# gear-genomics/tracy

Hardware: AMD Instinct MI355X
Metric: GCUPS (tracy align: Gotoh affine-gap DP cells per second, whole job) (higher is better)
Workload: dtype int16 (score sweeps) / int32 (tracebacks)

## Files before the change

### tracy_amd/csrc/pipe_kernels.h

```cpp
#ifndef TRACY_AMD_PIPE_KERNELS_H
#define TRACY_AMD_PIPE_KERNELS_H

#include <hip/hip_runtime.h>

#include "capi_internal.h"
#include "stream_plan.h"

namespace {
using namespace tracyhip;

__global__ __launch_bounds__(64) void trim_kernel(const uint8_t* __restrict__ ops, const uint64_t* __restrict__ ops_off,
                                                  const uint32_t* __restrict__ ops_len, const uint32_t* __restrict__ ref_len,
                                                  const uint8_t* __restrict__ forward, const uint32_t* __restrict__ trim_left,
                                                  const uint32_t* __restrict__ trim_right, uint32_t ntraces, TrimRec* __restrict__ out) {
  const uint32_t t = blockIdx.x;
  if (t >= ntraces) return;
  const uint8_t* o = ops + ops_off[t];
  const uint32_t L = ops_len[t];
  const uint32_t lane = threadIdx.x;
  int32_t s = -1, e = -1;
  for (uint32_t base = 0; base < L; base += 64) {
    const uint32_t j = base + lane;
    const bool hit = (j < L) && (o[L - 1 - j] != 'h');
    const unsigned long long m = __ballot(hit);
// ... 136 lines not shown
      b[j] = (uint8_t)c;
      if (c >= 4u) { f |= c >= 5u ? 2 : 4; any = true; }
    }
    if (cnt == kCqBytesPerThread) __builtin_memcpy(out + i0, b, kCqBytesPerThread);
    else for (uint32_t j = 0; j < cnt; ++j) out[i0 + j] = b[j];
    if (any && special) { special[i0 >> 8] = 1; special[(i0 + cnt - 1) >> 8] = 1; }
  }
  if (f) atomicOr(flag, f);
}
__global__ void cq_rows_kernel(const uint8_t* __restrict__ in, uint64_t n, int32_t* flag) {
  const uint64_t i0 = ((uint64_t)blockIdx.x * blockDim.x + threadIdx.x) * kCqBytesPerThread;
  if (i0 >= n) return;
  const uint32_t cnt = n - i0 < kCqBytesPerThread ? (uint32_t)(n - i0) : kCqBytesPerThread;
  uint8_t b[kCqBytesPerThread];
  if (cnt == kCqBytesPerThread) __builtin_memcpy(b, in + i0, kCqBytesPerThread);
  else for (uint32_t j = 0; j < cnt; ++j) b[j] = in[i0 + j];
  bool bad = false;
#pragma unroll
  for (uint32_t j = 0; j < kCqBytesPerThread; ++j)
    if (j < cnt && !cq_row_char(b[j])) bad = true;
  if (bad) atomicOr(flag, 1);
}

__device__ __forceinline__ uint32_t encode_word(uint32_t w, uint32_t cnt, bool& any_special, bool& invalid) {
  uint32_t codes = 0;
#pragma unroll
  for (uint32_t j = 0; j < 4u; ++j) {
    const uint8_t ch = (uint8_t)(w >> (8 * j));
    const uint8_t up = ch & 0xdfu;
    const uint32_t c = up == 'A' ? 0u : up == 'C' ? 1u : up == 'G' ? 2u : up == 'T' ? 3u : up == 'N' ? 4u : 5u;
    if (j < cnt) {
      invalid |= !(ch == 'A' || ch == 'C' || ch == 'G' || ch == 'T' || ch == 'N');
      any_special |= c >= 4u;
    }
    codes |= c << (8 * j);
  }
  return codes;
}
__global__ __launch_bounds__(256) void encode_codes_kernel(const uint8_t* __restrict__ in, uint8_t* __restrict__ out, uint64_t n,
                                                           uint8_t* __restrict__ special, int32_t* __restrict__ verr) {
  const uint64_t i0 = ((uint64_t)blockIdx.x * blockDim.x + threadIdx.x) * 16u;
  if (i0 >= n) return;
  bool any_special = false, invalid = false;
  if (n - i0 >= 16u) {
    uint32_t w[4];
    __builtin_memcpy(w, in + i0, 16);
#pragma unroll
    for (int q = 0; q < 4; ++q) w[q] = encode_word(w[q], 4u, any_special, invalid);
    __builtin_memcpy(out + i0, w, 16);
  } else {
    for (uint64_t i = i0; i < n; i += 4) {
      const uint32_t cnt = (n - i < 4u) ? (uint32_t)(n - i) : 4u;
      uint32_t w = 0;
      for (uint32_t j = 0; j < cnt; ++j) w |= (uint32_t)in[i + j] << (8 * j);
      const uint32_t c = encode_word(w, cnt, any_special, invalid);
      for (uint32_t j = 0; j < cnt; ++j) out[i + j] = (uint8_t)(c >> (8 * j));
    }
  }
  if (any_special) special[i0 >> 8] = 1;
  if (verr && invalid) atomicOr(verr, 4);
}

struct VoteDesc { uint64_t a1_off, a2_off; uint32_t stride, m, n, pad; };
constexpr int kVoteK = 11;
constexpr uint32_t kVoteBits = 1u << 16;
constexpr uint32_t kVotePiece = 65, kVoteTile = 64 * kVotePiece;
__device__ inline uint32_t vote_hash(uint32_t kmer) { return (kmer * 0x9E3779B1u) >> 16; }
__global__ __launch_bounds__(64) void kmer_vote_kernel(const VoteDesc* __restrict__ desc, const float* __restrict__ prof,
                                                       const uint8_t* __restrict__ codes, uint32_t* __restrict__ votes) {
  __shared__ uint32_t bm[2][kVoteBits / 32];
  __shared__ uint8_t cons[1040];
  __shared__ __attribute__((aligned(16))) uint8_t win[kVoteTile + 16];
  const VoteDesc d = desc[blockIdx.x];
  const uint32_t lane = threadIdx.x;
  uint32_t hf = 0, hr = 0;
  const uint32_t m = d.m < 1024u ? d.m : 1024u;
  if (m >= (uint32_t)kVoteK && d.n >= (uint32_t)kVoteK) {
    for (uint32_t i = lane; i < kVoteBits / 32; i += 64) { bm[0][i] = 0; bm[1][i] = 0; }
    constexpr uint32_t kCols = 8;
    for (uint32_t j0 = 0; j0 < m; j0 += 64 * kCols) {
      float v[kCols][4];
#pragma unroll
      for (uint32_t u = 0; u < kCols; ++u) {
// ... 83 lines not shown
```

### tracy_amd/csrc/pipeline.hip

```cpp
#include <hip/hip_runtime.h>

#include <algorithm>
#include <cstdlib>
#include <cstring>
#include <numeric>
#include <string>
#include <thread>
#include <vector>

#include "../../include/tracy_hip.h"
#include "capi_internal.h"
#include "launch.h"
#include "pipe_internal.h"
#include "pipe_kernels.h"
#include "stream_fields.h"

using namespace tracyhip;

namespace {
void reset_call_stats(tracyhip_ctx* ctx, uint32_t ntraces) {
  ctx->stats = tracyhip_call_stats{};
  ctx->stats.traces = ntraces;
  for (auto* l : ctx->lanes) l->stats = tracyhip_call_stats{};
}
// ... 719 lines not shown
  std::vector<B16TableDesc> td;
  bool b16 = false;
  OrientOut oo;
  std::vector<TrimRec> h_trim;
  void *d_final_sc = nullptr, *d_ops = nullptr, *d_olen = nullptr;
  uint64_t ops_total = 0;

  AlignRun(tracyhip_ctx* c, const tracyhip_align_job* j, const tracyhip_params* q, int m, const tracyhip_align_result* o)
      : ctx(c), job(j), prm(q), mem(m), out(o), nt(j->ntraces), sp(j->profiles), sr(j->refs), st(c->stream), p(*q), trims(trims_of(j)) {
    p.hfree = 1;
    p.vfree = 0;
  }

  int setup() {
    int rc;
    const uint64_t ep = seqset_extent(sp), er = seqset_extent(sr);
    if ((rc = stage_in(ctx, ctx->dev[DB_IN1], sp.data, ep * 4, mem, &d_prof))) return rc;
    if ((rc = stage_in(ctx, ctx->dev[DB_IN2], sr.data, er, mem, &d_ref))) return rc;
    HIP_TRY(ctx->dev[DB_ERR].ensure(kErrBytes));
    HIP_TRY(hipMemsetAsync(ctx->dev[DB_ERR].p, 0, kErrBytes, st));
    d_verr = static_cast<int32_t*>(ctx->dev[DB_ERR].p) + kErrVerdictWord;
    HIP_TRY(ctx->ensure_codes(er ? er : 1, st));
    if (er) {
      hipLaunchKernelGGL(encode_codes_kernel, dim3((unsigned)((er + 4095) / 4096)), dim3(256), 0, st, static_cast<const uint8_t*>(d_ref),
                         ctx->codes(), er, ctx->special_blocks(), job->oriented ? (int32_t*)nullptr : d_verr);
      HIP_TRY(hipGetLastError());
    }
    mf.resize(nt); mt.resize(nt); tl.resize(nt); rn.resize(nt); ridx.resize(nt);
    uint64_t max_mn = 0;
    for (uint32_t t = 0; t < nt; ++t) {
      ridx[t] = job->ref_index ? job->ref_index[t] : t;
      if (ridx[t] >= sr.count) return set_error(TRACYHIP_ERR_ARG, "ref_index[%u] out of range", t);
      mf[t] = sp.length[t];
      rn[t] = sr.length[ridx[t]];
      uint32_t l = trims.left(t), r = trims.right(t);
      if ((uint64_t)l + r >= mf[t]) { l = 0; r = 0; }
      tl[t] = l;
      mt[t] = mf[t] - (l + r);
      max_mn = std::max<uint64_t>(max_mn, (uint64_t)mf[t] + rn[t]);
    }
    if ((rc = check_params(&p, max_mn))) return rc;

    return TRACYHIP_OK;
  }

  int orient() {
    int rc;
// ... 572 lines not shown
      if ((rc = stage_in(ctx, buf(), bc.signal, sext * 4, mem, &d_sig))) return rc;
      if ((rc = stage_in(ctx, buf(), bc.bcpos, bext * 4, mem, &d_pos))) return rc;
    }
    for (uint32_t t = 0; t < nt; ++t) dext = std::max<uint64_t>(dext, out->dcp_offset[t] + 2ull * dp.maxindel + 2);
    if ((rc = io(bc.primary, bext, true, &d_pri))) return rc;
    if ((rc = io(bc.secondary, bext, true, &d_sec))) return rc;
    if ((rc = io(out->bp, sizeof(BreakpointOut) * (size_t)nt, false, &d_bp))) return rc;
    if ((rc = io(out->secdecomp, bext, false, &d_sd))) return rc;
    if ((rc = io(out->fractions, sizeof(double) * 2 * (size_t)nt, false, &d_fr))) return rc;
    if ((rc = io(out->dcp_indel, dext * 4, false, &d_di))) return rc;
    if ((rc = io(out->dcp_err, dext * 4, false, &d_de))) return rc;
    if (mem == TRACYHIP_MEM_HOST) {
      HIP_TRY(hipMemsetAsync(d_di, 0, dext * 4, st));
      HIP_TRY(hipMemsetAsync(d_de, 0, dext * 4, st));
    }
    if ((rc = io(out->dstatus, sizeof(DecompOut) * (size_t)nt, false, &d_dst))) return rc;
    if ((rc = io(out->score_trim, sizeof(int32_t) * (size_t)nt, false, &d_strim))) return rc;

    HIP_TRY(ctx->dev[DB_ERR].ensure(kErrBytes));
    HIP_TRY(hipMemsetAsync(ctx->dev[DB_ERR].p, 0, kErrBytes, st));
    HIP_TRY(ctx->ensure_codes(er ? er : 1, st));
    if (er) {
      int32_t* d_verr = static_cast<int32_t*>(ctx->dev[DB_ERR].p) + kErrVerdictWord;
      hipLaunchKernelGGL(encode_codes_kernel, dim3((unsigned)((er + 4095) / 4096)), dim3(256), 0, st, static_cast<const uint8_t*>(d_ref),
                         ctx->codes(), er, ctx->special_blocks(), job->oriented ? (int32_t*)nullptr : d_verr);
      HIP_TRY(hipGetLastError());
      int32_t herr = 0;
      HIP_TRY(hipMemcpyAsync(&herr, d_verr, sizeof(int32_t), hipMemcpyDeviceToHost, st));
      HIP_TRY(ctx_sync(ctx));
      if ((herr & 4) && !wildtype) return set_error(TRACYHIP_ERR_ARG, "reference windows must be upper-case [ACGTN] (loadSingleFasta, fasta.h:54-95)");
    }

    return TRACYHIP_OK;
  }

  int orientation() {
    int rc;
    stage_clock.mark("decompose.2_orientation");
    HIP_TRY(b_sc2.ensure(sizeof(int32_t) * 2 * (size_t)nt));
    h_sc2.assign(2 * (size_t)nt, 0);
    if (!given && !shared_stages) {
      DpProblem pb;
      DpProblemLease lease(ctx, pb);
      pb.mode = MODE_PROF; pb.a1_profile = true; pb.a2_profile = true; pb.d_a1 = d_prof; pb.d_a2 = d_refprof;
      pb.desc.resize(2 * (size_t)nt); pb.k.resize(2 * (size_t)nt);
      for (uint32_t t = 0; t < nt; ++t) {
        PairDesc d = qp_desc(t, true);
// ... 868 lines not shown
```

### tracy_amd/csrc/stream.hip

```cpp
#include <hip/hip_runtime.h>

#include <algorithm>
#include <cstring>
#include <numeric>
#include <string>
#include <type_traits>
#include <vector>

#include "../../include/tracy_hip.h"
#include "capi_internal.h"
#include "decompose_launch.h"
#include "launch.h"
#include "pipe_internal.h"
#include "pipe_kernels.h"
#include "stream_fields.h"
#include "stream_plan.h"

using namespace tracyhip;

#define TRY(expr) do { const int _rc = (expr); if (_rc) return _rc; } while (0)

namespace {

struct Arena {
// ... 10 lines not shown
  void take_into(T*& p, size_t count) { p = take<T>(count); }
};

__device__ __forceinline__ void s_count(unsigned long long* lc, int which, unsigned long long v = 1ull) { atomicAdd(lc + which, v); }
template <class Body>
__device__ __forceinline__ void with_counters(unsigned long long* cnt, Body body) {
  __shared__ unsigned long long lc[SC_COUNT];
  for (uint32_t i = threadIdx.x; i < (uint32_t)SC_COUNT; i += blockDim.x) lc[i] = 0;
  __syncthreads();
  body(lc);
  __syncthreads();
  for (uint32_t i = threadIdx.x; i < (uint32_t)SC_COUNT; i += blockDim.x)
    if (lc[i]) atomicAdd(cnt + i, lc[i]);
}
__device__ __forceinline__ void s_count_front(unsigned long long* lc, const FrontDesc& f) {
  const Credit c = front_credit(f.m_rest, f.n, kFrontK1, kFrontHalfW1);
  s_count(lc, SC_FRONT_CELLS, c.cells);
  s_count(lc, SC_FRONT_BYTES, c.bytes);
}

inline int queued_prio(const tracyhip_ctx* ctx, uint32_t tier) { return ctx->queue_prio >= tier ? 1 : 0; }

__global__ void s_expand_kernel(const SGeom* __restrict__ geom, uint32_t nt, VoteDesc* __restrict__ vd, RowMaxDesc* __restrict__ rm_rest,
                                RowMaxDesc* __restrict__ rm_trim, RowMaxDesc* __restrict__ rm_full, B16TableDesc* __restrict__ td) {
  const uint32_t t = blockIdx.x * blockDim.x + threadIdx.x;
  if (t >= nt) return;
  const SGeom G = geom[t];
  const uint64_t a1 = G.prof_off + G.tl;
  vd[t] = VoteDesc{a1, G.ref_off, G.mf, G.mt, G.rn, 0u};
  rm_rest[t] = RowMaxDesc{a1, G.mf, G.mt, kFrontRows};
  rm_trim[t] = RowMaxDesc{a1, G.mf, G.mt, 0u};
  if (rm_full) rm_full[t] = RowMaxDesc{G.prof_off, G.mf, G.mf, 0u};
  td[t] = B16TableDesc{G.prof_off, G.tab_off, G.mf, G.mf, G.tab_stride, 0u};
}

__device__ __forceinline__ PairDesc s_stage1_desc(const SGeom& G, uint32_t t, uint32_t nt, uint32_t o) {
  PairDesc d{};
  d.a1_off = G.prof_off + G.tl;
  d.a1_stride = G.mf;
  d.m = G.mt;
  d.a2_off = G.ref_off;
  d.n = G.rn;
  d.a2_stride = G.rn;
  d.out = o * nt + t;
  d.flags = o ? PAIR_A2_REVCOMP : 0u;
  d.lastrow_off = G.lr_off[o];
  return d;
}

__global__ void s_orient_plan_kernel(SParams p, const SGeom* __restrict__ geom, const uint32_t* __restrict__ votes, const int32_t* __restrict__ ub,
                                     const int32_t* __restrict__ ub1, PairDesc* __restrict__ full, PairDesc* __restrict__ pre,
                                     FrontDesc* __restrict__ fd, STrace* __restrict__ tr, unsigned long long* __restrict__ cnt) {
  with_counters(cnt, [&](unsigned long long* lc) {
  const uint32_t t = blockIdx.x * blockDim.x + threadIdx.x;
  if (t >= p.nt) return;
  const SGeom G = geom[t];
  const uint32_t R = kFrontRows;
  const SOrient o = s_orient_class(votes[2 * t], votes[2 * t + 1], G.mt, (G.flags & SG_FRONT_OK) != 0u, p.exact != 0u);
  const uint32_t g = o.g, cls = o.cls;
  PairDesc fa = s_skip_pair(t), fb = s_skip_pair(t), pa = s_skip_pair(t), pb = s_skip_pair(t);
  FrontDesc f{};
  f.flags = PAIR_SKIP;
  f.out = t;
  uint64_t cells = 0, bytes = 0, pcells = 0;
  const Credit full_c = sweep_pair_credit(G.mt, G.rn, true, false), pre_c = prefix_credit(G.mt, G.rn, R);
  const uint64_t full_cells = full_c.cells, pre_cells = pre_c.cells, full_bytes = full_c.bytes;
  if (cls == 0u) {
    pa = s_stage1_desc(G, t, p.nt, g);
    pa.flags |= PAIR_KEEP_ROW;
    pcells += pre_cells;
    if (p.exact) { fa = s_stage1_desc(G, t, p.nt, 1u - g); cells += full_cells; bytes += full_bytes; }
    else { pb = s_stage1_desc(G, t, p.nt, 1u - g); pcells += pre_cells; }
    f.row_off = G.lr_off[g];
    f.a2_off = G.ref_off;
    f.tab_off = G.tab_off + G.tl + R;
    f.tab_stride = G.tab_stride;
    f.m_rest = G.mt - R;
    f.n = G.rn;
    f.flags = g ? PAIR_A2_REVCOMP : 0u;
    f.R = R;
    f.rest = ub[t];
    f.tight = (p.ge <= -2 && ub1[t] <= ub[t]) ? (uint32_t)(ub[t] - ub1[t]) + 1u : 0u;
    s_count_front(lc, f);
  } else if (cls == 1u) {
    fa = s_stage1_desc(G, t, p.nt, g);
    fb = s_stage1_desc(G, t, p.nt, 1u - g);
    cells += 2 * full_cells; bytes += 2 * full_bytes;
  } else {
    fa = s_stage1_desc(G, t, p.nt, g);
    pb = s_stage1_desc(G, t, p.nt, 1u - g);
    cells += full_cells; pcells += pre_cells; bytes += full_bytes;
  }
  if (p.split_prefix) { s_count(lc, SC_FRONT_CELLS, pcells); s_count(lc, SC_FRONT_BYTES, pcells ? pre_c.bytes : 0ull); }
  else cells += pcells;
  full[G.full_a] = fa;
  full[G.full_b] = fb;
  pre[t] = pa;
  if (!p.exact) pre[p.nt + t] = pb;
  fd[t] = f;
  STrace S{};
  S.g = (uint8_t)g;
  S.cls = (uint8_t)cls;
  tr[t] = S;
  s_count(lc, SC_SWEEP_CELLS, cells);
  s_count(lc, SC_SWEEP_BYTES, bytes);
  });
}

__device__ __forceinline__ uint32_t s_front_result(uint32_t t, const FrontOut* __restrict__ fo1, const int32_t* __restrict__ fs1, const uint32_t* __restrict__ fe1,
                                                   const FrontOut* __restrict__ fo2, const int32_t* __restrict__ fs2, const uint32_t* __restrict__ fe2, int64_t* s_g) {
  if (fo1[t].ok) { *s_g = fs1[t]; return fe1[2 * t + 1] ? fe1[2 * t + 1] + fo1[t].shift : 0u; }
  if (fo2[t].ok) { *s_g = fs2[t]; return fe2[2 * t + 1] ? fe2[2 * t + 1] + fo2[t].shift : 0u; }
  return 0u;
}

__global__ void s_orient_early_kernel(SParams p, const FrontOut* __restrict__ fo1,
                                      const int32_t* __restrict__ fs1, const uint32_t* __restrict__ fe1, const FrontOut* __restrict__ fo2,
                                      const int32_t* __restrict__ fs2, const uint32_t* __restrict__ fe2, STrace* __restrict__ tr, int prio) {
  wave_prio(prio);
  const uint32_t t = blockIdx.x * blockDim.x + threadIdx.x;
  if (t >= p.nt) return;
  STrace S = tr[t];
  if (S.cls != 0u || !p.use_votes || !p.exact) return;
  const uint32_t g = S.g;
  int64_t s_g = 0;
  const uint32_t fce = s_front_result(t, fo1, fs1, fe1, fo2, fs2, fe2, &s_g);
  if (fce == 0u) return;
  if (g == 0u) S.sc[0] = (int32_t)s_g;
  else S.sc[1] = (int32_t)s_g;
// ... 577 lines not shown
  for (int b = 0; b < 4; ++b) { ak[b].index = sc.idx + (size_t)b * n; ak[b].count = count + b; }
  if (!quads) ak[3].npairs = 0;
  TRY(timing_begin(ctx, bl.kind == 0 ? TRACYHIP_TIMER_TRACE : TRACYHIP_TIMER_ORIGIN, 0, 0));
  bool large = false;
  HIP_TRY(launch_band16_counted(bl.kind, ak[0], ak[1], ak[2], ak[3], st, (ctx->b16_fork_ok && !ctx->knobs.no_fork) ? &ctx->b16_fork : nullptr,
                                ctx->knobs.b16_multi_max, &large));
  if (large) ++sc.large_stages;
  TRY(timing_end(ctx));
  return TRACYHIP_OK;
}

uint64_t band_words_cap(uint64_t rows, uint64_t npairs, uint64_t budget_left) {
  const uint64_t worst = rows * 131 + npairs * 10240;
  return std::max<uint64_t>(std::min(worst, budget_left / 2), 1ull << 20);
}
struct OrientStage {
  const void* d_prof;
  const int16_t* d_qp;
  int32_t* d_lastrow;
  bool exact;
  PairDesc* desc_trim;
  std::function<int()> filler;
  std::function<int()> early_tail;
};
int queue_orientation(tracyhip_ctx* ctx, const tracyhip_params& p, const SParams& sp, const StreamHost& h, StreamCommon& sc, const OrientStage& os) {
  hipStream_t st = ctx->stream;
  const uint32_t nt = h.nt;
  const dim3 g256((nt + 255) / 256), b256(256);
  const float* prof = static_cast<const float*>(os.d_prof);
  hipLaunchKernelGGL(s_expand_kernel, g256, b256, 0, st, sc.geom, nt, sc.vd, sc.rm_rest, sc.rm_trim, sc.rm_full, sc.td);
  HIP_TRY(hipGetLastError());
  const bool prep_fork = ctx->b16_fork_ok && !ctx->knobs.no_fork;
  hipStream_t sp1 = st;
  if (prep_fork) {
    HIP_TRY(hipEventRecord(ctx->b16_fork.forked, st));
    HIP_TRY(hipStreamWaitEvent(ctx->b16_fork.side[1], ctx->b16_fork.forked, 0));
    sp1 = ctx->b16_fork.side[1];
    ctx->stream = sp1;
  }
  {
    int rc = timing_begin(ctx, TRACYHIP_TIMER_MISC, 0, h.tab_tot * 2);
    hipError_t e = hipSuccess;
    if (!rc) {
      e = launch_b16_tables(sc.td, nt, os.d_prof, false, p.match, p.mismatch, sub_limit(&p), kTagShift, const_cast<int16_t*>(os.d_qp),
                            static_cast<int32_t*>(ctx->dev[DB_ERR].p), sp1);
      rc = timing_end(ctx);
    }
    ctx->stream = st;
    hipLaunchKernelGGL(rowmax_rest_kernel, dim3(nt), dim3(64), 0, sp1, sc.rm_rest, prof, (float)p.match, (float)p.mismatch, sc.ub, sc.ub1);
    hipLaunchKernelGGL(rowmax_rest_kernel, dim3(nt), dim3(64), 0, sp1, sc.rm_trim, prof, (float)p.match, (float)p.mismatch, sc.top_trim, (int32_t*)nullptr);
    if (sc.rm_full) hipLaunchKernelGGL(rowmax_rest_kernel, dim3(nt), dim3(64), 0, sp1, sc.rm_full, prof, (float)p.match, (float)p.mismatch, sc.top_full, (int32_t*)nullptr);
    hipLaunchKernelGGL(kmer_vote_kernel, dim3(nt), dim3(64), 0, st, sc.vd, prof, ctx->codes(), sc.votes);
    if (prep_fork) {
      HIP_TRY(hipEventRecord(ctx->b16_fork.joined[1], sp1));
      HIP_TRY(hipStreamWaitEvent(st, ctx->b16_fork.joined[1], 0));
    }
    if (rc) return rc;
    HIP_TRY(e);
  }
  hipLaunchKernelGGL(s_orient_plan_kernel, g256, b256, 0, st, sp, sc.geom, sc.votes, sc.ub, sc.ub1, sc.full, sc.pre, sc.fd, sc.tr, sc.cnt);
  HIP_TRY(hipGetLastError());
  DpArgs a = sweep_args(ctx, p, os.d_prof, ctx->codes(), sc.sc2, os.d_lastrow);
  if (!ctx->knobs.no_compact) a.special_blocks = ctx->special_blocks();
  if (sp.use_votes) { a.votes = sc.votes; a.vote_nt = nt; }
  DpArgs ap = a;
  ap.pairs = sc.pre;
  ap.votes = nullptr;
  const uint32_t npre_all = (os.exact ? 1u : 2u) * nt;
  auto front_tiers = [&]() -> int {
    TRY(timing_begin(ctx, TRACYHIP_TIMER_FRONT, 0, 0));
    const int rc = front_tiers_run(ctx, p, sc, nt, os.d_qp, ctx->codes(), reinterpret_cast<const uint32_t*>(os.d_lastrow), h.max_rest);
    const int rc2 = timing_end(ctx);
    return rc ? rc : rc2;
  };
  if (ctx->b16_fork_ok && !ctx->knobs.no_fork) {
    const B16Fork& fk = ctx->b16_fork;
    HIP_TRY(hipEventRecord(fk.forked, st));
    HIP_TRY(hipStreamWaitEvent(fk.side[0], fk.forked, 0));
    ctx->stream = fk.side[0];
    int rc = TRACYHIP_OK;
    {
      DpArgs af = a, apl = ap;
      launch_diag_periods(ctx, &p, h.classes[0].K, 0u, npre_all, true, af, apl);
      const uint32_t tall_min = (os.exact && !ctx->knobs.no_prefix_tall_beside) ? 0u : ctx->knobs.prefix_tall_min;
      if (launch_gotoh_ckpt_front(h.classes[0].K, af, 0u, apl, npre_all, fk.side[0], tall_min) != hipSuccess) rc = set_error(TRACYHIP_ERR_HIP, "prefix launch failed");
    }
    ctx->queue_prio = ctx->knobs.chain_prio;
    if (!rc) rc = front_tiers();
    if (!rc && os.early_tail) {
      hipLaunchKernelGGL(s_orient_early_kernel, g256, b256, 0, fk.side[0], sp, sc.fo1, sc.fs1, sc.fe1, sc.fo2, sc.fs2, sc.fe2, sc.tr, queued_prio(ctx, 1));
      if (hipGetLastError() != hipSuccess) rc = set_error(TRACYHIP_ERR_HIP, "early decision launch failed");
      else rc = os.early_tail();
    }
    ctx->queue_prio = 0;
    ctx->stream = st;
    HIP_TRY(hipEventRecord(fk.joined[0], fk.side[0]));
    if (rc) {
      HIP_TRY(hipStreamWaitEvent(st, fk.joined[0], 0));
      return rc;
    }
    if (ctx->knobs.sweeps_alone) HIP_TRY(hipStreamWaitEvent(st, fk.joined[0], 0));
    auto sweeps = [&]() -> int {
      for (const SweepClass& c : h.classes) {
        DpArgs af = a;
        af.pairs = sc.full + 2 * (size_t)c.lo;
        DpArgs apl = ap;
        launch_diag_periods(ctx, &p, c.K, 2 * (c.hi - c.lo), 0u, true, af, apl);
        TRY(timing_begin(ctx, TRACYHIP_TIMER_SCORE, 0, 0));
        const hipError_t e = launch_gotoh_ckpt_front(c.K, af, 2 * (c.hi - c.lo), apl, 0u, st, ctx->knobs.prefix_tall_min);
// ... 257 lines not shown
  uint64_t words_cap = 0;
  SParams spm{};
  dim3 g256, b256;
  const int16_t* d_qp = nullptr;
  int32_t* d_lastrow = nullptr;
  ReadBack rb;
  std::vector<uint32_t> dl;
  std::vector<uint64_t> sub_poff;
  std::vector<uint32_t> sub_plen, sub_ridx, sub_tl, sub_tr;

  template <class Job>
  StreamCall(tracyhip_ctx* c, const Job* j, const tracyhip_params* q, int m, StreamHost& h_)
      : ctx(c), prm(q), mem(m), kn(c->knobs), nt(j->ntraces), sp(j->profiles), sr(j->refs), st(c->stream), p(*q), trims(trims_of(j)),
        exact(j->strand_by_certificate == 0), host(m == TRACYHIP_MEM_HOST), h(h_), g256((j->ntraces + 255) / 256), b256(256) {
    p.hfree = 1;
    p.vfree = 0;
  }

  int size_ncap() {
    ncap = band_code_cap(h.maxmf + 200u);
    return band_lds_fits(ncap, 12, kBandLdsHard) ? TRACYHIP_OK : kStreamNo;
  }

  int encode_references(const uint8_t* refs, uint64_t er) {
    HIP_TRY(ctx->dev[DB_ERR].ensure(kErrBytes));
    HIP_TRY(hipMemsetAsync(ctx->dev[DB_ERR].p, 0, kErrBytes, st));
    int32_t* d_verr = static_cast<int32_t*>(ctx->dev[DB_ERR].p) + kErrVerdictWord;
    HIP_TRY(ctx->ensure_codes(er ? er : 1, st));
    if (er) {
      hipLaunchKernelGGL(encode_codes_kernel, dim3((unsigned)((er + 4095) / 4096)), dim3(256), 0, st, refs, ctx->codes(), er, ctx->special_blocks(), d_verr);
      HIP_TRY(hipGetLastError());
    }
    return TRACYHIP_OK;
  }

  int upload_records(StreamCommon& sc, void* d_own, size_t own_bytes) {
    HIP_TRY(hipMemcpyAsync(sc.geom, geom, sizeof(SGeom) * (size_t)nt, hipMemcpyHostToDevice, st));
    HIP_TRY(hipMemcpyAsync(d_own, geom + nt, own_bytes, hipMemcpyHostToDevice, st));
    HIP_TRY(hipMemsetAsync(sc.dead, 0, sizeof(uint32_t) * (size_t)nt, st));
    HIP_TRY(hipMemsetAsync(sc.cnt, 0, sizeof(unsigned long long) * SC_COUNT, st));
    HIP_TRY(hipMemsetAsync(sc.bstat, 0, sizeof(unsigned long long) * SB_COUNT * 8, st));
    sc.large_stages = 0;
    return TRACYHIP_OK;
  }

  void fill_params() {
    spm.match = p.match; spm.mismatch = p.mismatch; spm.go = p.go; spm.ge = p.ge; spm.nt = nt; spm.exact = exact ? 1u : 0u; spm.ncap = ncap - 8u;
    spm.use_votes = 1u;
    spm.split_prefix = kn.sweeps_alone ? 1u : 0u;
    d_qp = static_cast<const int16_t*>(ctx->dev[DB_B16TAB_PROFILE].p);
    d_lastrow = static_cast<int32_t*>(ctx->dev[DB_LASTROW].p);
  }

  template <class GiveUp>
  int await_verdict(GiveUp give_up) {
    HIP_TRY(ctx_sync(ctx));
    timing_collect(ctx);
    if (rb.herr[kErrVerdictWord] & 4) {
      (void)give_up(kStreamNo);
      return set_error(TRACYHIP_ERR_ARG, "reference windows must be upper-case [ACGTN] (loadSingleFasta, fasta.h:54-95)");
    }
    return give_up(stream_range_verdict(p, rb.herr, h));
  }

// ... 97 lines not shown
    A.layout(sizing, nt, exact, host, ops_bound);
    TRY(with_fresh_budget(ctx, [&](bool* from_cache) -> int {
      uint64_t budget = 0;
      TRY(workspace_budget(ctx, ctx->dev[DB_LASTROW].cap + ctx->dev[DB_BITS].cap + ctx->dev[DB_STREAM].cap + ctx->dev[DB_B16TAB_PROFILE].cap, &budget, from_cache));
      const uint64_t fixed = h.lr_tot * 4 + 64 + h.tab_tot * 2 + 64 + sizing.off;
      if (fixed > budget) return kStreamNo;
      words_cap = band_words_cap(rows_total, nt, budget - fixed);
      HIP_TRY(ctx->dev[DB_LASTROW].ensure(h.lr_tot * 4 + 64));
      HIP_TRY(ctx->dev[DB_B16TAB_PROFILE].ensure(h.tab_tot * sizeof(int16_t) + 64));
      HIP_TRY(ctx->dev[DB_BITS].ensure(words_cap + 64));
      HIP_TRY(ctx->dev[DB_STREAM].ensure(sizing.off + 256));
      return TRACYHIP_OK;
    }));
    Arena arena;
    arena.base = static_cast<char*>(ctx->dev[DB_STREAM].p);
    A.layout(arena, nt, exact, host, ops_bound);
    return TRACYHIP_OK;
  }

  int bind() {
    const uint64_t ep = seqset_extent(sp), er = seqset_extent(sr);
    TRY(stage_in(ctx, ctx->dev[DB_IN1], sp.data, ep * 4, mem, &d_prof));
    TRY(stage_in(ctx, ctx->dev[DB_IN2], sr.data, er, mem, &d_ref));
    TRY(encode_references(static_cast<const uint8_t*>(d_ref), er));
    std::memcpy(geom + nt, out->ops_offset, sizeof(uint64_t) * (size_t)nt);
    TRY(upload_records(A.sc, A.ops_off, sizeof(uint64_t) * (size_t)nt));
    fill_params();
    o = A.o;
    d_ops = A.ops;
    if (!host) { point_all<AlignFields>(o, *out); d_ops = out->ops; }
    return TRACYHIP_OK;
  }

  int queue_alignments(int early) {
    StreamCommon& sc = A.sc;
    hipStream_t s = ctx->stream;
    hipLaunchKernelGGL(s_prelim_plan_kernel, g256, b256, 0, s, spm, 0, early, sc.geom, sc.tr, sc.ce, sc.top_trim, sc.dead, sc.cand, sc.kc, queued_prio(ctx, 2));
    HIP_TRY(hipGetLastError());
    BandStageArgs b1;
    b1.kind = 1; b1.qp = d_qp; b1.codes = ctx->codes(); b1.ends = sc.ends; b1.code_cap = ncap; b1.hfree = 1;
    TRY(band_stage(ctx, p, sc, nt, nt, 0, b1, ~0ull));
    hipLaunchKernelGGL(s_align_final_plan_kernel, g256, b256, 0, s, spm, early, sc.geom, sc.tr, sc.ends, sc.dead, sc.cand, sc.kc, sc.cnt, queued_prio(ctx, 2));
    HIP_TRY(hipGetLastError());
    BandStageArgs b2;
    b2.kind = 0; b2.qp = d_qp; b2.codes = ctx->codes(); b2.scores = o.score_final; b2.ops = d_ops; b2.ops_off = A.ops_off; b2.ops_len = o.ops_len; b2.code_cap = ncap;
    b2.hfree = 1;
    return band_stage(ctx, p, sc, nt, nt, 1, b2, words_cap);
  }

  int queue_stages() {
    StreamCommon& sc = A.sc;
    OrientStage os{d_prof, d_qp, d_lastrow, exact, nullptr};
    if (!kn.no_early_tail && exact) os.early_tail = [this]() { return queue_alignments(1); };
    TRY(queue_orientation(ctx, p, spm, h, sc, os));
    TRY(queue_alignments(0));
    hipLaunchKernelGGL(s_align_finish_kernel, g256, b256, 0, st, spm, sc.tr, sc.top_full, sc.dead, o, sc.cnt);
    HIP_TRY(hipGetLastError());
    return TRACYHIP_OK;
  }

  int read_back() {
    TRY(rb.carve(ctx, nt, host ? sizeof(uint32_t) * (size_t)nt : 0));
    hlen = static_cast<uint32_t*>(rb.extra);
    TRY(rb.queue_verdict(ctx, st));
    TRY(rb.queue_counters(A.sc, nt, st));
    if (host) HIP_TRY(hipMemcpyAsync(hlen, o.slice_len, sizeof(uint32_t) * (size_t)nt, hipMemcpyDeviceToHost, st));
    TRY(await_verdict([](int rc) { return rc; }));
    static const int stage_timer[2] = {TRACYHIP_TIMER_ORIGIN, TRACYHIP_TIMER_TRACE};
    static const DeadReason reasons[] = {{SD_FRONT, "front"}, {SD_STRAND, "strand"}, {SD_LOSER_WON, "loser won"}, {SD_JUNK, "junk"}, {SD_PRELIM_BAND, "prelim band"},
                                         {SD_FINAL_BAND, "final band"}, {SD_FINAL_CHECK, "final check"}, {SD_MEM, "mem"}, {SD_SHAPE, "shape"}};
    list_dead("align", A.sc, stage_timer, reasons);
    return TRACYHIP_OK;
  }

  int redo_dead_traces() {
    if (dl.empty()) return TRACYHIP_OK;
// ... 561 lines not shown
    d_pri = bc.primary; d_sec = bc.secondary; d_sd = out->secdecomp;
    d_di = out->dcp_indel; d_de = out->dcp_err;
    o = A.o;
    for (int k = 0; k < 3; ++k) d_opsK[k] = out->ops[k];
    if (host) {
      auto up = [&](void* dev, const void* src, size_t bytes) -> int {
        if (bytes) HIP_TRY(hipMemcpyAsync(dev, src, bytes, hipMemcpyHostToDevice, st));
        return TRACYHIP_OK;
      };
      TRY(up(A.in_prof, sp.data, z.ep * 4)); TRY(up(A.in_ref, sr.data, z.er));
      if (bc.peaks) { TRY(up(A.peaks, bc.peaks, z.bext * 16)); d_peaks = A.peaks; }
      else { TRY(up(A.in_sig, bc.signal, z.sext * 4)); TRY(up(A.in_pos, bc.bcpos, z.bext * 4)); }
      TRY(up(A.pri, bc.primary, z.bext)); TRY(up(A.sec, bc.secondary, z.bext));
      d_prof = A.in_prof; d_ref = A.in_ref; d_sig = A.in_sig; d_pos = A.in_pos; d_pri = A.pri; d_sec = A.sec; d_sd = A.secdecomp;
      d_di = A.dcp_indel; d_de = A.dcp_err;
      HIP_TRY(hipMemsetAsync(d_di, 0, z.dext * 4, st)); HIP_TRY(hipMemsetAsync(d_de, 0, z.dext * 4, st));
      for (int k = 0; k < 3; ++k) d_opsK[k] = A.ops[k];
    } else {
      point_all<DecompFields>(o, *out);
    }
    HIP_TRY(hipMemcpyAsync(A.pri_bak, d_pri, z.bext, hipMemcpyDeviceToDevice, st));
    HIP_TRY(hipMemcpyAsync(A.sec_bak, d_sec, z.bext, hipMemcpyDeviceToDevice, st));

    if (!encoded_early) TRY(encode_references(d_ref, z.er));
    TRY(upload_records(sc, A.geomd, sizeof(SGeomD) * (size_t)nt));

    fill_params();
    spd.bext = z.bext;
    spd.best = (int32_t)std::max<int64_t>(std::max<int64_t>(p.match, p.mismatch), 0);

    return TRACYHIP_OK;
  }

  int queue_trace_stages() {
    StreamCommon& sc = A.sc;
    OrientStage os{d_prof, d_qp, d_lastrow, exact, A.desc_trim};
    hipLaunchKernelGGL(s_expand_d_kernel, g256, b256, 0, st, sc.geom, A.geomd, nt, z.bext, A.bpd, A.rowsd, A.dd, A.bcd, A.atd, A.off1, A.aops_off, A.ops2_off,
                       (uint64_t)(reinterpret_cast<uintptr_t>(d_opsK[1]) - reinterpret_cast<uintptr_t>(d_opsK[0])));
    HIP_TRY(hipGetLastError());
    if (build_peaks && ctx->b16_fork_ok && !ctx->knobs.no_fork) {
      const B16Fork& fk = ctx->b16_fork;
      HIP_TRY(hipEventRecord(fk.forked, st));
      HIP_TRY(hipStreamWaitEvent(fk.side[3], fk.forked, 0));
      ctx->stream = fk.side[3];
      const int rcp = launch_peaks(ctx, A.bcd, nt, maxbc, d_sig, d_pos, A.peaks);
      ctx->stream = st;
      HIP_TRY(hipEventRecord(fk.ready[1], fk.side[3]));
      peaks_forked = true;
      if (rcp) return rcp;
      build_peaks = false;
    }
    bp_early = ctx->b16_fork_ok && !ctx->knobs.no_fork;
    if (bp_early)
      os.filler = [&]() -> int {
        TRY(launch_breakpoint(ctx, A.bpd, nt, h.maxmt, d_prof, reinterpret_cast<BreakpointOut*>(o.bp)));
        return encode_windows_cq();
      };
    TRY(give_up(queue_orientation(ctx, p, spm, h, sc, os)));
    hipLaunchKernelGGL(s_prelim_plan_kernel, g256, b256, 0, st, spm, 1, 0, sc.geom, sc.tr, sc.ce, sc.top_trim, sc.dead, sc.cand, sc.kc, 0);
    HIP_TRY(hipGetLastError());
    BandStageArgs b0;
    b0.kind = 0; b0.qp = d_qp; b0.codes = ctx->codes(); b0.scores = A.sb; b0.ops = A.ops1; b0.ops_off = A.off1; b0.ops_len = A.len1; b0.code_cap = ncap; b0.hfree = 1;
    TRY(band_stage(ctx, p, sc, nt, nt, 0, b0, words_cap));
    hipLaunchKernelGGL(s_prelim_check_kernel, g256, b256, 0, st, spm, sc.tr, A.sb, A.len1, sc.kc, o.score_trim, sc.dead, sc.cnt);
    HIP_TRY(hipGetLastError());
    BreakpointOut* bpo = reinterpret_cast<BreakpointOut*>(o.bp);
    if (!bp_early) TRY(launch_breakpoint(ctx, A.bpd, nt, h.maxmt, d_prof, bpo));
    {
      RowsArgs ra{};
      ra.pairs = A.desc_trim;
      ra.a1 = d_prof; ra.a2 = d_ref;
      ra.a1_profile = 1; ra.a2_profile = 0; ra.a2_revcomp_flag = 1; ra.a2_onehot = 1;
      ra.ops = A.ops1; ra.ops_off = A.off1; ra.ops_len = A.len1;
      ra.rows0 = A.rows0; ra.rows1 = A.rows1;
      ra.npairs = nt;
      static_assert(offsetof(BreakpointOut, indelshift) == 0 && sizeof(BreakpointOut) == 16, "layout");
      ra.row0_gaps_only = reinterpret_cast<const int32_t*>(bpo);
      ra.row0_gaps_only_stride = 4;
      HIP_TRY(launch_alignment_rows(ra, st));
    }
// ... 202 lines not shown
```

Measured before the change: 19480.

## Overlap reference encoding with rowmax prep and fold memsets into expand kernel

The reference-encoding kernel becomes a grid-stride, SWAR byte-permute encoder with an aligned body, unaligned head and tail, and wave-level ballots for special-block and validity flags. It is now launched inside the orientation stage, after the rowmax side-stream work is queued, so it overlaps that work instead of running up front. The three memsets for dead, cnt and bstat are folded into s_expand_kernel, which moves to upload time. The ub/ub1-dependent FrontDesc fields are written by a new kernel on the side stream, which removes the join before orientation planning; the join moves to the prefix stream instead. The stream and event reordering adds a risk of ordering bugs on FrontDesc between the two writers.

```diff
diff --git a/tracy_amd/csrc/pipe_kernels.h b/tracy_amd/csrc/pipe_kernels.h
--- a/tracy_amd/csrc/pipe_kernels.h
+++ b/tracy_amd/csrc/pipe_kernels.h
@@ -182,43 +182,78 @@
   if (bad) atomicOr(flag, 1);
 }
 
-__device__ __forceinline__ uint32_t encode_word(uint32_t w, uint32_t cnt, bool& any_special, bool& invalid) {
-  uint32_t codes = 0;
-#pragma unroll
-  for (uint32_t j = 0; j < 4u; ++j) {
-    const uint8_t ch = (uint8_t)(w >> (8 * j));
-    const uint8_t up = ch & 0xdfu;
-    const uint32_t c = up == 'A' ? 0u : up == 'C' ? 1u : up == 'G' ? 2u : up == 'T' ? 3u : up == 'N' ? 4u : 5u;
-    if (j < cnt) {
-      invalid |= !(ch == 'A' || ch == 'C' || ch == 'G' || ch == 'T' || ch == 'N');
-      any_special |= c >= 4u;
-    }
-    codes |= c << (8 * j);
-  }
-  return codes;
+__device__ __forceinline__ uint32_t encode_byte(uint8_t ch, bool& invalid) {
+  const uint8_t up = ch & 0xdfu;
+  invalid |= !(ch == 'A' || ch == 'C' || ch == 'G' || ch == 'T' || ch == 'N');
+  return up == 'A' ? 0u : up == 'C' ? 1u : up == 'G' ? 2u : up == 'T' ? 3u : up == 'N' ? 4u : 5u;
+}
+__device__ __forceinline__ uint32_t encode_word(uint32_t w, uint32_t& nonletter, uint32_t& seen, uint32_t& raw) {
+  const uint32_t h = (w >> 1) & 0x07070707u;
+  const uint32_t letter = __builtin_amdgcn_perm(0x4effffffu, 0x47544341u, h);
+  const uint32_t code = __builtin_amdgcn_perm(0x04050505u, 0x02030100u, h);
+  const uint32_t x = (w & 0xdfdfdfdfu) ^ letter;
+  const uint32_t nz = (((x & 0x7f7f7f7fu) + 0x7f7f7f7fu) | x) & 0x80808080u;
+  const uint32_t full = (nz << 1) - (nz >> 7);
+  const uint32_t c = (code & ~full) | (0x05050505u & full);
+  nonletter |= nz;
+  seen |= c;
+  raw |= w;
+  return c;
+}
+constexpr uint32_t kEncPieces = 4, kEncThreads = 256, kEncMaxBlocks = 1024;
+inline uint32_t encode_codes_blocks(uint64_t n) {
+  const uint64_t want = (n / 16u + (uint64_t)kEncThreads * kEncPieces - 1) / ((uint64_t)kEncThreads * kEncPieces);
+  return (uint32_t)(want < 1 ? 1 : want > kEncMaxBlocks ? kEncMaxBlocks : want);
 }
 __global__ __launch_bounds__(256) void encode_codes_kernel(const uint8_t* __restrict__ in, uint8_t* __restrict__ out, uint64_t n,
                                                            uint8_t* __restrict__ special, int32_t* __restrict__ verr) {
-  const uint64_t i0 = ((uint64_t)blockIdx.x * blockDim.x + threadIdx.x) * 16u;
-  if (i0 >= n) return;
-  bool any_special = false, invalid = false;
-  if (n - i0 >= 16u) {
-    uint32_t w[4];
-    __builtin_memcpy(w, in + i0, 16);
-#pragma unroll
-    for (int q = 0; q < 4; ++q) w[q] = encode_word(w[q], 4u, any_special, invalid);
-    __builtin_memcpy(out + i0, w, 16);
-  } else {
-    for (uint64_t i = i0; i < n; i += 4) {
-      const uint32_t cnt = (n - i < 4u) ? (uint32_t)(n - i) : 4u;
-      uint32_t w = 0;
-      for (uint32_t j = 0; j < cnt; ++j) w |= (uint32_t)in[i + j] << (8 * j);
-      const uint32_t c = encode_word(w, cnt, any_special, invalid);
-      for (uint32_t j = 0; j < cnt; ++j) out[i + j] = (uint8_t)(c >> (8 * j));
-    }
-  }
-  if (any_special) special[i0 >> 8] = 1;
-  if (verr && invalid) atomicOr(verr, 4);
+  const uint64_t gid = (uint64_t)blockIdx.x * blockDim.x + threadIdx.x, nthreads = (uint64_t)gridDim.x * blockDim.x;
+  const uint64_t to_boundary = (16u - (uint32_t)(reinterpret_cast<uintptr_t>(out) & 15u)) & 15u;
+  const uint64_t head = to_boundary < n ? to_boundary : n;
+  const uint64_t np = (n - head) / 16u;
+  bool invalid = false;
+  if (gid < 32u) {
+    const uint64_t tail0 = head + 16u * np;
+    const uint64_t i = gid < 16u ? gid : tail0 + (gid - 16u);
+    if (gid < 16u ? i < head : i < n) {
+      const uint32_t c = encode_byte(in[i], invalid);
+      out[i] = (uint8_t)c;
+      if (c >= 4u) special[i >> 8] = 1;
+    }
+  }
+  for (uint64_t q0 = gid; q0 < np; q0 += nthreads * kEncPieces) {
+    uint4 v[kEncPieces];
+#pragma unroll
+    for (uint32_t k = 0; k < kEncPieces; ++k) {
+      const uint64_t q = q0 + k * nthreads;
+      if (q < np) __builtin_memcpy(&v[k], in + head + 16u * q, 16);
+    }
+#pragma unroll
+    for (uint32_t k = 0; k < kEncPieces; ++k) {
+      const uint64_t q = q0 + k * nthreads;
+      uint32_t nonletter = 0, seen = 0, raw = 0;
+      if (q < np) {
+        v[k].x = encode_word(v[k].x, nonletter, seen, raw);
+        v[k].y = encode_word(v[k].y, nonletter, seen, raw);
+        v[k].z = encode_word(v[k].z, nonletter, seen, raw);
+        v[k].w = encode_word(v[k].w, nonletter, seen, raw);
+        *reinterpret_cast<uint4*>(out + head + 16u * q) = v[k];
+      }
+      invalid |= (nonletter | (raw & 0x20202020u)) != 0u;
+      const unsigned long long sp = __ballot((seen & 0x04040404u) != 0u);
+      if (sp) {
+        const uint32_t lane = threadIdx.x & 63u;
+        const uint64_t b0 = head + 16u * q;
+        if (head == 0u) {
+          if ((lane & 15u) == 0u && ((sp >> lane) & 0xffffull)) special[b0 >> 8] = 1;
+        } else if ((sp >> lane) & 1ull) {
+          special[b0 >> 8] = 1;
+          special[(b0 + 15u) >> 8] = 1;
+        }
+      }
+    }
+  }
+  if (verr && __ballot(invalid) && (threadIdx.x & 63u) == 0u) atomicOr(verr, 4);
 }
 
 struct VoteDesc { uint64_t a1_off, a2_off; uint32_t stride, m, n, pad; };
diff --git a/tracy_amd/csrc/pipeline.hip b/tracy_amd/csrc/pipeline.hip
--- a/tracy_amd/csrc/pipeline.hip
+++ b/tracy_amd/csrc/pipeline.hip
@@ -765,7 +765,7 @@
     d_verr = static_cast<int32_t*>(ctx->dev[DB_ERR].p) + kErrVerdictWord;
     HIP_TRY(ctx->ensure_codes(er ? er : 1, st));
     if (er) {
-      hipLaunchKernelGGL(encode_codes_kernel, dim3((unsigned)((er + 4095) / 4096)), dim3(256), 0, st, static_cast<const uint8_t*>(d_ref),
+      hipLaunchKernelGGL(encode_codes_kernel, dim3(encode_codes_blocks(er)), dim3(kEncThreads), 0, st, static_cast<const uint8_t*>(d_ref),
                          ctx->codes(), er, ctx->special_blocks(), job->oriented ? (int32_t*)nullptr : d_verr);
       HIP_TRY(hipGetLastError());
     }
@@ -1384,7 +1384,7 @@
     HIP_TRY(ctx->ensure_codes(er ? er : 1, st));
     if (er) {
       int32_t* d_verr = static_cast<int32_t*>(ctx->dev[DB_ERR].p) + kErrVerdictWord;
-      hipLaunchKernelGGL(encode_codes_kernel, dim3((unsigned)((er + 4095) / 4096)), dim3(256), 0, st, static_cast<const uint8_t*>(d_ref),
+      hipLaunchKernelGGL(encode_codes_kernel, dim3(encode_codes_blocks(er)), dim3(kEncThreads), 0, st, static_cast<const uint8_t*>(d_ref),
                          ctx->codes(), er, ctx->special_blocks(), job->oriented ? (int32_t*)nullptr : d_verr);
       HIP_TRY(hipGetLastError());
       int32_t herr = 0;
diff --git a/tracy_amd/csrc/stream.hip b/tracy_amd/csrc/stream.hip
--- a/tracy_amd/csrc/stream.hip
+++ b/tracy_amd/csrc/stream.hip
@@ -56,9 +56,15 @@
 inline int queued_prio(const tracyhip_ctx* ctx, uint32_t tier) { return ctx->queue_prio >= tier ? 1 : 0; }
 
 __global__ void s_expand_kernel(const SGeom* __restrict__ geom, uint32_t nt, VoteDesc* __restrict__ vd, RowMaxDesc* __restrict__ rm_rest,
-                                RowMaxDesc* __restrict__ rm_trim, RowMaxDesc* __restrict__ rm_full, B16TableDesc* __restrict__ td) {
+                                RowMaxDesc* __restrict__ rm_trim, RowMaxDesc* __restrict__ rm_full, B16TableDesc* __restrict__ td,
+                                uint32_t* __restrict__ dead, unsigned long long* __restrict__ cnt, unsigned long long* __restrict__ bstat) {
+  if (blockIdx.x == 0) {
+    for (uint32_t i = threadIdx.x; i < (uint32_t)SC_COUNT; i += blockDim.x) cnt[i] = 0;
+    for (uint32_t i = threadIdx.x; i < (uint32_t)SB_COUNT * 8u; i += blockDim.x) bstat[i] = 0;
+  }
   const uint32_t t = blockIdx.x * blockDim.x + threadIdx.x;
   if (t >= nt) return;
+  dead[t] = 0;
   const SGeom G = geom[t];
   const uint64_t a1 = G.prof_off + G.tl;
   vd[t] = VoteDesc{a1, G.ref_off, G.mf, G.mt, G.rn, 0u};
@@ -82,9 +88,9 @@
   return d;
 }
 
-__global__ void s_orient_plan_kernel(SParams p, const SGeom* __restrict__ geom, const uint32_t* __restrict__ votes, const int32_t* __restrict__ ub,
-                                     const int32_t* __restrict__ ub1, PairDesc* __restrict__ full, PairDesc* __restrict__ pre,
-                                     FrontDesc* __restrict__ fd, STrace* __restrict__ tr, unsigned long long* __restrict__ cnt) {
+__global__ void s_orient_plan_kernel(SParams p, const SGeom* __restrict__ geom, const uint32_t* __restrict__ votes, PairDesc* __restrict__ full,
+                                     PairDesc* __restrict__ pre, FrontDesc* __restrict__ fd, STrace* __restrict__ tr,
+                                     unsigned long long* __restrict__ cnt) {
   with_counters(cnt, [&](unsigned long long* lc) {
   const uint32_t t = blockIdx.x * blockDim.x + threadIdx.x;
   if (t >= p.nt) return;
@@ -113,8 +119,6 @@
     f.n = G.rn;
     f.flags = g ? PAIR_A2_REVCOMP : 0u;
     f.R = R;
-    f.rest = ub[t];
-    f.tight = (p.ge <= -2 && ub1[t] <= ub[t]) ? (uint32_t)(ub[t] - ub1[t]) + 1u : 0u;
     s_count_front(lc, f);
   } else if (cls == 1u) {
     fa = s_stage1_desc(G, t, p.nt, g);
@@ -131,7 +135,11 @@
   full[G.full_b] = fb;
   pre[t] = pa;
   if (!p.exact) pre[p.nt + t] = pb;
-  fd[t] = f;
+  {
+    FrontDesc& d = fd[t];
+    d.row_off = f.row_off; d.a2_off = f.a2_off; d.tab_off = f.tab_off; d.tab_stride = f.tab_stride; d.m_rest = f.m_rest; d.n = f.n;
+    d.flags = f.flags; d.out = f.out; d.R = f.R;
+  }
   STrace S{};
   S.g = (uint8_t)g;
   S.cls = (uint8_t)cls;
@@ -139,6 +147,13 @@
   s_count(lc, SC_SWEEP_CELLS, cells);
   s_count(lc, SC_SWEEP_BYTES, bytes);
   });
+}
+
+__global__ void s_front_rest_kernel(SParams p, const int32_t* __restrict__ ub, const int32_t* __restrict__ ub1, FrontDesc* __restrict__ fd) {
+  const uint32_t t = blockIdx.x * blockDim.x + threadIdx.x;
+  if (t >= p.nt) return;
+  fd[t].rest = ub[t];
+  fd[t].tight = (p.ge <= -2 && ub1[t] <= ub[t]) ? (uint32_t)(ub[t] - ub1[t]) + 1u : 0u;
 }
 
 __device__ __forceinline__ uint32_t s_front_result(uint32_t t, const FrontOut* __restrict__ fo1, const int32_t* __restrict__ fs1, const uint32_t* __restrict__ fe1,
@@ -762,14 +777,13 @@
   PairDesc* desc_trim;
   std::function<int()> filler;
   std::function<int()> early_tail;
+  std::function<int()> encode;
 };
 int queue_orientation(tracyhip_ctx* ctx, const tracyhip_params& p, const SParams& sp, const StreamHost& h, StreamCommon& sc, const OrientStage& os) {
   hipStream_t st = ctx->stream;
   const uint32_t nt = h.nt;
   const dim3 g256((nt + 255) / 256), b256(256);
   const float* prof = static_cast<const float*>(os.d_prof);
-  hipLaunchKernelGGL(s_expand_kernel, g256, b256, 0, st, sc.geom, nt, sc.vd, sc.rm_rest, sc.rm_trim, sc.rm_full, sc.td);
-  HIP_TRY(hipGetLastError());
   const bool prep_fork = ctx->b16_fork_ok && !ctx->knobs.no_fork;
   hipStream_t sp1 = st;
   if (prep_fork) {
@@ -788,18 +802,23 @@
     }
     ctx->stream = st;
     hipLaunchKernelGGL(rowmax_rest_kernel, dim3(nt), dim3(64), 0, sp1, sc.rm_rest, prof, (float)p.match, (float)p.mismatch, sc.ub, sc.ub1);
+    hipLaunchKernelGGL(s_front_rest_kernel, g256, b256, 0, sp1, sp, sc.ub, sc.ub1, sc.fd);
     hipLaunchKernelGGL(rowmax_rest_kernel, dim3(nt), dim3(64), 0, sp1, sc.rm_trim, prof, (float)p.match, (float)p.mismatch, sc.top_trim, (int32_t*)nullptr);
     if (sc.rm_full) hipLaunchKernelGGL(rowmax_rest_kernel, dim3(nt), dim3(64), 0, sp1, sc.rm_full, prof, (float)p.match, (float)p.mismatch, sc.top_full, (int32_t*)nullptr);
+    if (prep_fork) HIP_TRY(hipEventRecord(ctx->b16_fork.joined[1], sp1));
+    if (!rc && e == hipSuccess && os.encode) rc = os.encode();
+    if (rc || e != hipSuccess) {
+      if (prep_fork) HIP_TRY(hipStreamWaitEvent(st, ctx->b16_fork.joined[1], 0));
+      if (rc) return rc;
+      HIP_TRY(e);
+    }
     hipLaunchKernelGGL(kmer_vote_kernel, dim3(nt), dim3(64), 0, st, sc.vd, prof, ctx->codes(), sc.votes);
-    if (prep_fork) {
-      HIP_TRY(hipEventRecord(ctx->b16_fork.joined[1], sp1));
-      HIP_TRY(hipStreamWaitEvent(st, ctx->b16_fork.joined[1], 0));
-    }
-    if (rc) return rc;
+  }
+  hipLaunchKernelGGL(s_orient_plan_kernel, g256, b256, 0, st, sp, sc.geom, sc.votes, sc.full, sc.pre, sc.fd, sc.tr, sc.cnt);
+  if (const hipError_t e = hipGetLastError(); e != hipSuccess) {
+    if (prep_fork) (void)hipStreamWaitEvent(st, ctx->b16_fork.joined[1], 0);
     HIP_TRY(e);
   }
-  hipLaunchKernelGGL(s_orient_plan_kernel, g256, b256, 0, st, sp, sc.geom, sc.votes, sc.ub, sc.ub1, sc.full, sc.pre, sc.fd, sc.tr, sc.cnt);
-  HIP_TRY(hipGetLastError());
   DpArgs a = sweep_args(ctx, p, os.d_prof, ctx->codes(), sc.sc2, os.d_lastrow);
   if (!ctx->knobs.no_compact) a.special_blocks = ctx->special_blocks();
   if (sp.use_votes) { a.votes = sc.votes; a.vote_nt = nt; }
@@ -825,6 +844,7 @@
       const uint32_t tall_min = (os.exact && !ctx->knobs.no_prefix_tall_beside) ? 0u : ctx->knobs.prefix_tall_min;
       if (launch_gotoh_ckpt_front(h.classes[0].K, af, 0u, apl, npre_all, fk.side[0], tall_min) != hipSuccess) rc = set_error(TRACYHIP_ERR_HIP, "prefix launch failed");
     }
+    if (hipStreamWaitEvent(fk.side[0], fk.joined[1], 0) != hipSuccess && !rc) rc = set_error(TRACYHIP_ERR_HIP, "joining the table stream failed");
     ctx->queue_prio = ctx->knobs.chain_prio;
     if (!rc) rc = front_tiers();
     if (!rc && os.early_tail) {
@@ -1128,24 +1148,29 @@
     return band_lds_fits(ncap, 12, kBandLdsHard) ? TRACYHIP_OK : kStreamNo;
   }
 
-  int encode_references(const uint8_t* refs, uint64_t er) {
+  int prepare_codes(uint64_t er) {
     HIP_TRY(ctx->dev[DB_ERR].ensure(kErrBytes));
     HIP_TRY(hipMemsetAsync(ctx->dev[DB_ERR].p, 0, kErrBytes, st));
+    HIP_TRY(ctx->ensure_codes(er ? er : 1, st));
+    return TRACYHIP_OK;
+  }
+  int launch_encoder(const uint8_t* refs, uint64_t er) {
+    if (!er) return TRACYHIP_OK;
     int32_t* d_verr = static_cast<int32_t*>(ctx->dev[DB_ERR].p) + kErrVerdictWord;
-    HIP_TRY(ctx->ensure_codes(er ? er : 1, st));
-    if (er) {
-      hipLaunchKernelGGL(encode_codes_kernel, dim3((unsigned)((er + 4095) / 4096)), dim3(256), 0, st, refs, ctx->codes(), er, ctx->special_blocks(), d_verr);
-      HIP_TRY(hipGetLastError());
-    }
-    return TRACYHIP_OK;
+    hipLaunchKernelGGL(encode_codes_kernel, dim3(encode_codes_blocks(er)), dim3(kEncThreads), 0, ctx->stream, refs, ctx->codes(), er, ctx->special_blocks(), d_verr);
+    HIP_TRY(hipGetLastError());
+    return TRACYHIP_OK;
+  }
+  int encode_references(const uint8_t* refs, uint64_t er) {
+    TRY(prepare_codes(er));
+    return launch_encoder(refs, er);
   }
 
   int upload_records(StreamCommon& sc, void* d_own, size_t own_bytes) {
     HIP_TRY(hipMemcpyAsync(sc.geom, geom, sizeof(SGeom) * (size_t)nt, hipMemcpyHostToDevice, st));
     HIP_TRY(hipMemcpyAsync(d_own, geom + nt, own_bytes, hipMemcpyHostToDevice, st));
-    HIP_TRY(hipMemsetAsync(sc.dead, 0, sizeof(uint32_t) * (size_t)nt, st));
-    HIP_TRY(hipMemsetAsync(sc.cnt, 0, sizeof(unsigned long long) * SC_COUNT, st));
-    HIP_TRY(hipMemsetAsync(sc.bstat, 0, sizeof(unsigned long long) * SB_COUNT * 8, st));
+    hipLaunchKernelGGL(s_expand_kernel, g256, b256, 0, st, sc.geom, nt, sc.vd, sc.rm_rest, sc.rm_trim, sc.rm_full, sc.td, sc.dead, sc.cnt, sc.bstat);
+    HIP_TRY(hipGetLastError());
     sc.large_stages = 0;
     return TRACYHIP_OK;
   }
@@ -1289,7 +1314,7 @@
     const uint64_t ep = seqset_extent(sp), er = seqset_extent(sr);
     TRY(stage_in(ctx, ctx->dev[DB_IN1], sp.data, ep * 4, mem, &d_prof));
     TRY(stage_in(ctx, ctx->dev[DB_IN2], sr.data, er, mem, &d_ref));
-    TRY(encode_references(static_cast<const uint8_t*>(d_ref), er));
+    TRY(prepare_codes(er));
     std::memcpy(geom + nt, out->ops_offset, sizeof(uint64_t) * (size_t)nt);
     TRY(upload_records(A.sc, A.ops_off, sizeof(uint64_t) * (size_t)nt));
     fill_params();
@@ -1319,6 +1344,7 @@
     StreamCommon& sc = A.sc;
     OrientStage os{d_prof, d_qp, d_lastrow, exact, nullptr};
     if (!kn.no_early_tail && exact) os.early_tail = [this]() { return queue_alignments(1); };
+    os.encode = [this]() { return launch_encoder(static_cast<const uint8_t*>(d_ref), seqset_extent(sr)); };
     TRY(queue_orientation(ctx, p, spm, h, sc, os));
     TRY(queue_alignments(0));
     hipLaunchKernelGGL(s_align_finish_kernel, g256, b256, 0, st, spm, sc.tr, sc.top_full, sc.dead, o, sc.cnt);
@@ -1926,7 +1952,7 @@
     HIP_TRY(hipMemcpyAsync(A.pri_bak, d_pri, z.bext, hipMemcpyDeviceToDevice, st));
     HIP_TRY(hipMemcpyAsync(A.sec_bak, d_sec, z.bext, hipMemcpyDeviceToDevice, st));
 
-    if (!encoded_early) TRY(encode_references(d_ref, z.er));
+    if (!encoded_early) TRY(prepare_codes(z.er));
     TRY(upload_records(sc, A.geomd, sizeof(SGeomD) * (size_t)nt));
 
     fill_params();
@@ -1960,6 +1986,7 @@
         TRY(launch_breakpoint(ctx, A.bpd, nt, h.maxmt, d_prof, reinterpret_cast<BreakpointOut*>(o.bp)));
         return encode_windows_cq();
       };
+    if (!encoded_early) os.encode = [this]() { return launch_encoder(d_ref, z.er); };
     TRY(give_up(queue_orientation(ctx, p, spm, h, sc, os)));
     hipLaunchKernelGGL(s_prelim_plan_kernel, g256, b256, 0, st, spm, 1, 0, sc.geom, sc.tr, sc.ce, sc.top_trim, sc.dead, sc.cand, sc.kc, 0);
     HIP_TRY(hipGetLastError());
```

Result: faster. 19750, median of 6 (+1.4%).
